# zkh2018/ethsnarks

Hardware: AMD Instinct MI355X
Metric: groth16_proofs_per_sec (higher is better)
Workload: dtype u32 (8-limb 254-bit Montgomery integers)

## Files before the change

### ethsnarks_amd/csrc/bn254.hpp

```cpp
#pragma once
#include "common.hpp"
#include <stdint.h>
#if defined(__HIP_DEVICE_COMPILE__) && !defined(ZK_NO_ASM)
#include "fips_asm.hpp"
#endif

#ifndef ZK_HD
#define ZK_HD __host__ __device__ __forceinline__
#endif
#define ZK_HD_NOINLINE __host__ __device__ __attribute__((noinline))

namespace zk {

struct alignas(16) fe { uint32_t l[8]; };

struct FrParams {
    static ZK_HD constexpr uint32_t p(int i) {
        constexpr uint32_t v[8] = {0xf0000001u, 0x43e1f593u, 0x79b97091u, 0x2833e848u, 0x8181585du, 0xb85045b6u, 0xe131a029u, 0x30644e72u};
        return v[i];
    }
    static ZK_HD constexpr uint32_t one(int i) {
        constexpr uint32_t v[8] = {0x4ffffffbu, 0xac96341cu, 0x9f60cd29u, 0x36fc7695u, 0x7879462eu, 0x666ea36fu, 0x9a07df2fu, 0x0e0a77c1u};
        return v[i];
    }
// ... 335 lines not shown
#endif
    static ZK_HD void lmul_pair(const fe &a, const fe &b, const fe &c, const fe &d, fe &r0, fe &r1) { lmul_x2(a, b, c, d, r0, r1); }
    static ZK_HD void lsqr_pair(const fe &a, const fe &b, fe &r0, fe &r1) { lmul_pair(a, a, b, b, r0, r1); }
    static ZK_HD fe lsqr(const fe &a) { return lmul(a, a); }
    static ZK_HD fe ldbl(const fe &a) { return ladd(a, a); }
    static ZK_HD fe lneg(const fe &a) { return lsub(zero(), a); }
#if defined(__HIP_DEVICE_COMPILE__) && !defined(ZK_NO_ASM)
    static __device__ __forceinline__ fe lneg_op(const fe &a) {
        fe pp, d;
#pragma unroll
        for (int i = 0; i < 8; i++) pp.l[i] = (P::p(i) << 1) | (i ? P::p(i - 1) >> 31 : 0u);
        fips::sub8(d.l, pp.l, a.l);
        return d;
    }
#else
    static ZK_HD fe lneg_op(const fe &a) { return lneg(a); }
#endif
    static ZK_HD fe lneg_yop(const fe &a) { return lneg(a); }
    static ZK_HD fe qsel(uint32_t ql, const fe &a, const fe &b, const fe &c, const fe &d) {
        fe r; const bool odd = ql & 1u, hi = ql & 2u;
#pragma unroll
        for (int i = 0; i < 8; i++) { const uint32_t x = odd ? b.l[i] : a.l[i], y = odd ? d.l[i] : c.l[i]; r.l[i] = hi ? y : x; }
        return r;
    }
#if defined(__HIP_DEVICE_COMPILE__) && !defined(ZK_NO_ASM)
    template <int S> static __device__ __forceinline__ fe qbcast(const fe &v) {
        fe r;
#pragma unroll
        for (int i = 0; i < 8; i++) r.l[i] = (uint32_t)__builtin_amdgcn_update_dpp(0, (int)v.l[i], S * 0x55, 0xf, 0xf, false);
        return r;
    }
#endif
    static ZK_HD fe canon(const fe &a) { return reduce_once(a); }

    static ZK_HD fe to_mont(const fe &a) { fe r2; for (int i = 0; i < 8; i++) r2.l[i] = P::r2(i); return mul(a, r2); }
    static ZK_HD fe from_mont(const fe &a) { fe o = zero(); o.l[0] = 1; return mul(a, o); }

    static ZK_HD fe pow(const fe &a, const uint32_t e[8]) {
        fe acc = one(), base = a;
        for (int i = 0; i < 256; i++) {
            if ((e[i >> 5] >> (i & 31)) & 1) acc = mul(acc, base);
            base = sqr(base);
        }
        return acc;
    }
    static ZK_HD fe pow_u64(const fe &a, uint64_t e) {
        fe acc = one(), base = a;
        while (e) { if (e & 1) acc = mul(acc, base); base = sqr(base); e >>= 1; }
        return acc;
    }
    static ZK_HD fe inv(const fe &a) {
        uint32_t e[8];
        for (int i = 0; i < 8; i++) e[i] = P::p(i);
        e[0] -= 2;
        return pow(a, e);
    }
    static ZK_HD fe from_u64(uint64_t v) { fe t = zero(); t.l[0] = (uint32_t)v; t.l[1] = (uint32_t)(v >> 32); return to_mont(t); }
};

typedef Field<FrParams> Fr;
typedef Field<FqParams> Fq;

struct alignas(16) fe2 { fe c0, c1; };

struct Fq2 {
    typedef fe2 elem;
    static ZK_HD fe2 zero() { fe2 r; r.c0 = Fq::zero(); r.c1 = Fq::zero(); return r; }
    static ZK_HD fe2 one() { fe2 r; r.c0 = Fq::one(); r.c1 = Fq::zero(); return r; }
    static ZK_HD bool is_zero(const fe2 &a) { return Fq::is_zero(a.c0) && Fq::is_zero(a.c1); }
    static ZK_HD bool eq(const fe2 &a, const fe2 &b) { return Fq::eq(a.c0, b.c0) && Fq::eq(a.c1, b.c1); }
    static ZK_HD fe2 add(const fe2 &a, const fe2 &b) { fe2 r; r.c0 = Fq::add(a.c0, b.c0); r.c1 = Fq::add(a.c1, b.c1); return r; }
    static ZK_HD fe2 sub(const fe2 &a, const fe2 &b) { fe2 r; r.c0 = Fq::sub(a.c0, b.c0); r.c1 = Fq::sub(a.c1, b.c1); return r; }
    static ZK_HD fe2 neg(const fe2 &a) { fe2 r; r.c0 = Fq::neg(a.c0); r.c1 = Fq::neg(a.c1); return r; }
    static ZK_HD fe2 dbl(const fe2 &a) { return add(a, a); }
    static ZK_HD fe2 mul(const fe2 &a, const fe2 &b) {
        fe v0 = Fq::mul(a.c0, b.c0), v1 = Fq::mul(a.c1, b.c1);
        fe s = Fq::mul(Fq::add(a.c0, a.c1), Fq::add(b.c0, b.c1));
        fe2 r; r.c0 = Fq::sub(v0, v1); r.c1 = Fq::sub(Fq::sub(s, v0), v1); return r;
    }
    static ZK_HD fe2 sqr(const fe2 &a) {
        fe p = Fq::mul(a.c0, a.c1);
        fe2 r; r.c0 = Fq::mul(Fq::add(a.c0, a.c1), Fq::sub(a.c0, a.c1)); r.c1 = Fq::add(p, p); return r;
    }
    static ZK_HD bool lis_zero(const fe2 &a) { return Fq::lis_zero(a.c0) && Fq::lis_zero(a.c1); }
    static ZK_HD fe2 ladd(const fe2 &a, const fe2 &b) { fe2 r; r.c0 = Fq::ladd(a.c0, b.c0); r.c1 = Fq::ladd(a.c1, b.c1); return r; }
    static ZK_HD fe2 lsub(const fe2 &a, const fe2 &b) { fe2 r; r.c0 = Fq::lsub(a.c0, b.c0); r.c1 = Fq::lsub(a.c1, b.c1); return r; }
    static ZK_HD fe2 lneg(const fe2 &a) { fe2 r; r.c0 = Fq::lneg(a.c0); r.c1 = Fq::lneg(a.c1); return r; }
    static ZK_HD fe2 lneg_op(const fe2 &a) { fe2 r; r.c0 = Fq::lneg_op(a.c0); r.c1 = Fq::lneg_op(a.c1); return r; }
    static ZK_HD fe2 lneg_yop(const fe2 &a) { return lneg_op(a); }
    static ZK_HD fe2 ldbl(const fe2 &a) { return ladd(a, a); }
    static ZK_HD fe2 lmul(const fe2 &a, const fe2 &b) {
        fe2 r;
        r.c0 = Fq::lmul2(a.c0, b.c0, a.c1, Fq::lneg_op(b.c1));
        r.c1 = Fq::lmul2(a.c0, b.c1, a.c1, b.c0);
        return r;
    }
    static constexpr bool PAIRS = false;
    static ZK_HD void lmul_pair(const fe2 &a, const fe2 &b, const fe2 &c, const fe2 &d, fe2 &r0, fe2 &r1) { r0 = lmul(a, b); r1 = lmul(c, d); }
    static ZK_HD void lsqr_pair(const fe2 &a, const fe2 &b, fe2 &r0, fe2 &r1) { r0 = lsqr(a); r1 = lsqr(b); }
    static ZK_HD fe2 lmul2(const fe2 &a, const fe2 &b, const fe2 &c, const fe2 &d) {
        fe2 r;
        r.c0 = Fq::lmul4(a.c0, b.c0, a.c1, Fq::lneg_op(b.c1), c.c0, d.c0, c.c1, Fq::lneg_op(d.c1));
        r.c1 = Fq::lmul4(a.c0, b.c1, a.c1, b.c0, c.c0, d.c1, c.c1, d.c0);
        return r;
    }
    static ZK_HD fe2 lsqr(const fe2 &a) {
        fe p = Fq::lmul(a.c0, a.c1);
        fe2 r; r.c0 = Fq::lmul(Fq::ladd(a.c0, a.c1), Fq::lsub(a.c0, a.c1)); r.c1 = Fq::ladd(p, p); return r;
    }
    static ZK_HD fe2 canon(const fe2 &a) { fe2 r; r.c0 = Fq::canon(a.c0); r.c1 = Fq::canon(a.c1); return r; }
    static ZK_HD fe2 qsel(uint32_t ql, const fe2 &a, const fe2 &b, const fe2 &c, const fe2 &d) {
        fe2 r; r.c0 = Fq::qsel(ql, a.c0, b.c0, c.c0, d.c0); r.c1 = Fq::qsel(ql, a.c1, b.c1, c.c1, d.c1); return r;
    }
#if defined(__HIP_DEVICE_COMPILE__) && !defined(ZK_NO_ASM)
    template <int S> static __device__ __forceinline__ fe2 qbcast(const fe2 &v) { fe2 r; r.c0 = Fq::qbcast<S>(v.c0); r.c1 = Fq::qbcast<S>(v.c1); return r; }
#endif
    static ZK_HD fe2 inv(const fe2 &a) {
        fe n = Fq::inv(Fq::add(Fq::sqr(a.c0), Fq::sqr(a.c1)));
        fe2 r; r.c0 = Fq::mul(a.c0, n); r.c1 = Fq::neg(Fq::mul(a.c1, n)); return r;
    }
};

template <class F>
struct Curve {
    typedef typename F::elem E;
    static constexpr int WAVES_PER_SIMD = sizeof(E) > 32 ? 2 : 4;
    static constexpr int WAVES_PER_SIMD_PAIRS = sizeof(E) > 32 ? 2 : 3;
    struct alignas(16) Affine { E x, y; };
    struct alignas(16) XYZZ { E X, Y, ZZ, ZZZ; };

    static ZK_HD bool is_inf(const Affine &p) { return F::lis_zero(p.x) && F::lis_zero(p.y); }
    static ZK_HD bool is_inf(const XYZZ &p) { return F::lis_zero(p.ZZ); }
    static ZK_HD XYZZ infinity() { XYZZ r; r.X = F::zero(); r.Y = F::zero(); r.ZZ = F::zero(); r.ZZZ = F::zero(); return r; }
    static ZK_HD Affine aff_infinity() { Affine r; r.x = F::zero(); r.y = F::zero(); return r; }
    static ZK_HD XYZZ from_affine(const Affine &p) {
        if (is_inf(p)) return infinity();
        XYZZ r; r.X = p.x; r.Y = p.y; r.ZZ = F::one(); r.ZZZ = F::one(); return r;
    }
    static ZK_HD Affine neg(const Affine &p) { Affine r; r.x = p.x; r.y = F::lneg(p.y); return r; }
    static ZK_HD XYZZ neg(const XYZZ &p) { XYZZ r = p; r.Y = F::lneg(p.Y); return r; }

    static ZK_HD XYZZ dbl_affine(const Affine &p) {
        if (is_inf(p)) return infinity();
        E U = F::ldbl(p.y), V = F::lsqr(U), W = F::lmul(U, V), S = F::lmul(p.x, V);
        E xx = F::lsqr(p.x), M = F::ladd(F::ldbl(xx), xx);
        XYZZ r;
        r.X = F::lsub(F::lsqr(M), F::ldbl(S));
        r.Y = F::lmul2(M, F::lsub(S, r.X), W, F::lneg_yop(p.y));
        r.ZZ = V; r.ZZZ = W;
        return r;
    }
    static ZK_HD XYZZ dbl(const XYZZ &p) {
        if (is_inf(p)) return p;
        E U = F::ldbl(p.Y), V = F::lsqr(U), W = F::lmul(U, V), S = F::lmul(p.X, V);
        E xx = F::lsqr(p.X), M = F::ladd(F::ldbl(xx), xx);
        XYZZ r;
        r.X = F::lsub(F::lsqr(M), F::ldbl(S));
        r.Y = F::lmul2(M, F::lsub(S, r.X), W, F::lneg_yop(p.Y));
        r.ZZ = F::lmul(V, p.ZZ); r.ZZZ = F::lmul(W, p.ZZZ);
        return r;
    }
    static ZK_HD XYZZ madd(const XYZZ &p, const Affine &q) {
        if (is_inf(q)) return p;
        if (is_inf(p)) { XYZZ r; r.X = q.x; r.Y = q.y; r.ZZ = F::one(); r.ZZZ = F::one(); return r; }
        E U2 = F::lmul(q.x, p.ZZ), S2 = F::lmul(q.y, p.ZZZ);
        E Pd = F::lsub(U2, p.X), R = F::lsub(S2, p.Y);
        if (F::lis_zero(Pd)) {
            if (F::lis_zero(R)) return dbl_affine(q);
            return infinity();
        }
        XYZZ r;
        const E PP = F::lsqr(Pd);
        r.ZZ = F::lmul(p.ZZ, PP);
        const E Q = F::lmul(p.X, PP), PPP = F::lmul(Pd, PP);
        r.ZZZ = F::lmul(p.ZZZ, PPP);
        r.X = F::lsub(F::lsub(F::lsqr(R), PPP), F::ldbl(Q));
        r.Y = F::lmul2(R, F::lsub(Q, r.X), F::lneg_yop(p.Y), PPP);
        return r;
    }
    static ZK_HD XYZZ madd_pairs(const XYZZ &p, const Affine &q) {
        if constexpr (!F::PAIRS) return madd(p, q);
        else {
        if (is_inf(q)) return p;
        if (is_inf(p)) { XYZZ r; r.X = q.x; r.Y = q.y; r.ZZ = F::one(); r.ZZZ = F::one(); return r; }
        E U2, S2;
        F::lmul_pair(q.x, p.ZZ, q.y, p.ZZZ, U2, S2);
        E Pd = F::lsub(U2, p.X), R = F::lsub(S2, p.Y);
        if (F::lis_zero(Pd)) {
            if (F::lis_zero(R)) return dbl_affine(q);
            return infinity();
        }
        XYZZ r;
        E PP, RR, Q, PPP;
        F::lsqr_pair(Pd, R, PP, RR);
        F::lmul_pair(p.X, PP, Pd, PP, Q, PPP);
        F::lmul_pair(p.ZZ, PP, p.ZZZ, PPP, r.ZZ, r.ZZZ);
        r.X = F::lsub(F::lsub(RR, PPP), F::ldbl(Q));
        r.Y = F::lmul2(R, F::lsub(Q, r.X), F::lneg_yop(p.Y), PPP);
        return r;
        }
    }
    static ZK_HD XYZZ add(const XYZZ &p, const XYZZ &q) {
        if (is_inf(p)) return q;
        if (is_inf(q)) return p;
        E U1 = F::lmul(p.X, q.ZZ), U2 = F::lmul(q.X, p.ZZ);
        E S1 = F::lmul(p.Y, q.ZZZ), S2 = F::lmul(q.Y, p.ZZZ);
        E Pd = F::lsub(U2, U1), R = F::lsub(S2, S1);
        if (F::lis_zero(Pd)) {
            if (F::lis_zero(R)) return dbl(p);
            return infinity();
        }
        E PP = F::lsqr(Pd), PPP = F::lmul(Pd, PP), Q = F::lmul(U1, PP);
        XYZZ r;
        r.X = F::lsub(F::lsub(F::lsqr(R), PPP), F::ldbl(Q));
        r.Y = F::lmul2(R, F::lsub(Q, r.X), F::lneg_yop(S1), PPP);
        r.ZZ = F::lmul(F::lmul(p.ZZ, q.ZZ), PP); r.ZZZ = F::lmul(F::lmul(p.ZZZ, q.ZZZ), PPP);
        return r;
    }
#if defined(__HIP_DEVICE_COMPILE__) && !defined(ZK_NO_ASM)
#define ZK_QB(S, v) F::template qbcast<S>(v)
    static __device__ __forceinline__ XYZZ dbl_q(const XYZZ &p, uint32_t ql) {
        if (is_inf(p)) return p;
        const E U = F::ldbl(p.Y);
        E a = F::qsel(ql, U, p.X, U, U);
        E t = F::lmul(a, a);
        const E V = ZK_QB(0, t), xx = ZK_QB(1, t), M = F::ladd(F::ldbl(xx), xx);
        t = F::lmul(F::qsel(ql, U, p.X, M, V), F::qsel(ql, V, V, M, p.ZZ));
        const E W = ZK_QB(0, t), S = ZK_QB(1, t), MM = ZK_QB(2, t);
        XYZZ r; r.ZZ = ZK_QB(3, t);
        r.X = F::lsub(MM, F::ldbl(S));
        t = F::lmul(F::qsel(ql, M, W, W, W), F::qsel(ql, F::lsub(S, r.X), p.Y, p.ZZZ, p.ZZZ));
        r.Y = F::lsub(ZK_QB(0, t), ZK_QB(1, t)); r.ZZZ = ZK_QB(2, t);
        return r;
    }
    static __device__ __forceinline__ XYZZ add_q(const XYZZ &p, const XYZZ &q, uint32_t ql) {
        if (is_inf(p)) return q;
        if (is_inf(q)) return p;
        E t = F::lmul(F::qsel(ql, p.X, q.X, p.Y, q.Y), F::qsel(ql, q.ZZ, p.ZZ, q.ZZZ, p.ZZZ));
        const E U1 = ZK_QB(0, t), U2 = ZK_QB(1, t), S1 = ZK_QB(2, t), S2 = ZK_QB(3, t);
        const E Pd = F::lsub(U2, U1), R = F::lsub(S2, S1);
        if (F::lis_zero(Pd)) {
            if (F::lis_zero(R)) return dbl_q(p, ql);
            return infinity();
        }
        t = F::lmul(F::qsel(ql, Pd, R, p.ZZ, p.ZZZ), F::qsel(ql, Pd, R, q.ZZ, q.ZZZ));
        const E PP = ZK_QB(0, t), RR = ZK_QB(1, t), ZZ12 = ZK_QB(2, t), ZZZ12 = ZK_QB(3, t);
        t = F::lmul(F::qsel(ql, Pd, U1, ZZ12, ZZ12), PP);
        const E PPP = ZK_QB(0, t), Q = ZK_QB(1, t);
        XYZZ r; r.ZZ = ZK_QB(2, t);
        r.X = F::lsub(F::lsub(RR, PPP), F::ldbl(Q));
        t = F::lmul(F::qsel(ql, R, S1, ZZZ12, ZZZ12), F::qsel(ql, F::lsub(Q, r.X), PPP, PPP, PPP));
        r.Y = F::lsub(ZK_QB(0, t), ZK_QB(1, t)); r.ZZZ = ZK_QB(2, t);
        return r;
    }
    static __device__ __forceinline__ XYZZ madd_q(const XYZZ &p, const Affine &q, uint32_t ql) {
        if (is_inf(q)) return p;
        if (is_inf(p)) { XYZZ r; r.X = q.x; r.Y = q.y; r.ZZ = F::one(); r.ZZZ = F::one(); return r; }
        E t = F::lmul(F::qsel(ql, q.x, q.y, q.x, q.y), F::qsel(ql, p.ZZ, p.ZZZ, p.ZZ, p.ZZZ));
        const E Pd = F::lsub(ZK_QB(0, t), p.X), R = F::lsub(ZK_QB(1, t), p.Y);
        if (F::lis_zero(Pd)) {
            if (F::lis_zero(R)) return dbl_affine(q);
            return infinity();
        }
        E a = F::qsel(ql, Pd, R, Pd, R);
        t = F::lmul(a, a);
        const E PP = ZK_QB(0, t), RR = ZK_QB(1, t);
        t = F::lmul(F::qsel(ql, Pd, p.X, p.ZZ, p.ZZ), PP);
        const E PPP = ZK_QB(0, t), Q = ZK_QB(1, t);
        XYZZ r; r.ZZ = ZK_QB(2, t);
        r.X = F::lsub(F::lsub(RR, PPP), F::ldbl(Q));
        t = F::lmul(F::qsel(ql, R, p.Y, p.ZZZ, p.ZZZ), F::qsel(ql, F::lsub(Q, r.X), PPP, PPP, PPP));
        r.Y = F::lsub(ZK_QB(0, t), ZK_QB(1, t)); r.ZZZ = ZK_QB(2, t);
        return r;
    }
#undef ZK_QB
#else
    static ZK_HD XYZZ dbl_q(const XYZZ &p, uint32_t) { return dbl(p); }
    static ZK_HD XYZZ add_q(const XYZZ &p, const XYZZ &q, uint32_t) { return add(p, q); }
    static ZK_HD XYZZ madd_q(const XYZZ &p, const Affine &q, uint32_t) { return madd(p, q); }
#endif
    template <int Q> static ZK_HD XYZZ addQ(const XYZZ &p, const XYZZ &q, uint32_t ql) { if constexpr (Q == 4) return add_q(p, q, ql); else return add(p, q); }
    template <int Q> static ZK_HD XYZZ dblQ(const XYZZ &p, uint32_t ql) { if constexpr (Q == 4) return dbl_q(p, ql); else return dbl(p); }
    template <int Q> static ZK_HD XYZZ maddQ(const XYZZ &p, const Affine &q, uint32_t ql) { if constexpr (Q == 4) return madd_q(p, q, ql); else return madd(p, q); }
    template <int Q> static ZK_HD XYZZ maddV(const XYZZ &p, const Affine &q, uint32_t ql) { if constexpr (Q == 2) return madd_pairs(p, q); else return maddQ<Q>(p, q, ql); }

    static ZK_HD XYZZ canon(const XYZZ &p) { XYZZ r; r.X = F::canon(p.X); r.Y = F::canon(p.Y); r.ZZ = F::canon(p.ZZ); r.ZZZ = F::canon(p.ZZZ); return r; }
    static ZK_HD Affine to_affine(const XYZZ &p) {
        if (is_inf(p)) return aff_infinity();
        const XYZZ c = canon(p);
        E i = F::inv(F::mul(c.ZZ, c.ZZZ));
        E izz = F::mul(i, c.ZZZ), izzz = F::mul(i, c.ZZ);
        Affine r; r.x = F::mul(c.X, izz); r.y = F::mul(c.Y, izzz); return r;
    }
};

typedef Curve<Fq> G1;
typedef Curve<Fq2> G2;

}
```

### ethsnarks_amd/csrc/msm.hpp

```cpp
#pragma once
#include "bn254.hpp"
#include "common.hpp"
#include <stdlib.h>

namespace zk {

constexpr uint32_t MSM_SEG_MIN = 32;
constexpr uint32_t MSM_SEG_MIN_SMALL = 8;
constexpr uint32_t MSM_SEG_MAX = 48;
constexpr uint32_t MSM_HEAVY = 64;
constexpr uint32_t MSM_TREE = 256;
constexpr uint32_t MSM_HEAVY_GRID = 256;

constexpr uint32_t SORT_THREADS = 256;
constexpr uint32_t SORT_FINE_THREADS = 1024;
constexpr uint32_t SORT_MAX_CB = 256;
constexpr uint32_t SORT_MAX_FB = 4096;
constexpr uint32_t SORT_STAGE = 7680;
static_assert(SORT_MAX_CB == SORT_THREADS, "k_sort_partition_staged: one coarse bin per thread");

struct SortShape {
    uint32_t cb, fb, fine_bits, groups, per_group;
    void set(uint32_t n, uint32_t nb, uint32_t W = 15) {
        per_group = 512;
        while (per_group > 32 && (uint64_t)per_group * W > SORT_STAGE) per_group >>= 1;
        if (const char *e = getenv("ZK_SORT_PER_GROUP")) { int v = atoi(e); if (v >= 64) per_group = (uint32_t)v; }
        resize(n, nb);
    }
    void resize(uint32_t n, uint32_t nb) {
        fine_bits = 0; while (((nb + (1u << fine_bits) - 1) >> fine_bits) > SORT_MAX_CB) fine_bits++;
        fb = 1u << fine_bits;
        cb = (nb + fb - 1) >> fine_bits;
        groups = (n + per_group - 1) / per_group; if (!groups) groups = 1;
    }
};

struct ChunkRule {
    uint32_t slots = 1, seg_min = MSM_SEG_MIN, seg_max = MSM_SEG_MAX;
    ZK_HD uint32_t len(uint32_t total) const {
        if ((uint64_t)seg_min * slots >= total) return seg_min;
        const uint64_t per_round = (uint64_t)seg_max * slots;
        const uint64_t rounds = (total + per_round - 1) / per_round, lanes = rounds * slots;
        const uint32_t seg = (uint32_t)((total + lanes - 1) / lanes);
        return seg < seg_min ? seg_min : seg;
    }
    uint64_t max_chunks(uint64_t entries_bound) const { return entries_bound / seg_max + slots + 1; }
};
inline uint32_t msm_machine_threads(uint32_t waves_per_simd) {
#ifdef ZK_EMUL
    return 32 * waves_per_simd;
#else
    int dev = 0, cus = 0;
    if (hipGetDevice(&dev) != hipSuccess || hipDeviceGetAttribute(&cus, hipDeviceAttributeMultiprocessorCount, dev) != hipSuccess || cus <= 0) cus = 256;
    return (uint32_t)cus * 4u * waves_per_simd * 64u;
#endif
}

struct MsmShape {
    uint32_t n = 0, c = 0, W = 0, nb = 0;
    uint32_t plog = 0;
    ZK_HD uint32_t planes() const { return 1u << plog; }
    ZK_HD uint32_t rows() const { return (W + planes() - 1) >> plog; }
    ZK_HD uint32_t lo_bits() const { return c / 2; }
    ZK_HD uint32_t hi_bits() const { return (c - 1) - c / 2; }
    ChunkRule chunk;
    uint32_t quad = 1;
    uint32_t quad_acc = 1;
    bool acc_pairs = false;
    uint32_t rowcol_seg = 16;
    static uint32_t pick_c(uint32_t n, uint32_t batch = 1) {
        for (uint32_t c = 17; c > 2; c--) {
            const uint64_t entries = (uint64_t)n * (254 / c + 1);
            const uint64_t floor_c = c >= 16 ? 2 * MSM_SEG_MIN - 1 : MSM_SEG_MIN;
            uint64_t per_bucket = floor_c;
            if (batch > 1) {
                per_bucket = 32 * entries * batch / 1482910;
                if (per_bucket > 100) per_bucket = 100;
                if (per_bucket < floor_c) per_bucket = floor_c;
            }
            if (entries >= (per_bucket << (c - 1))) return c;
        }
        return 2;
    }
    void set(uint32_t n_, uint32_t c_, uint32_t batch = 1, uint32_t plog_ = 0) {
        plog = plog_;
        n = n_; c = c_ ? c_ : pick_c(n_, batch ? batch : 1);
        if (c < 2) c = 2;
        if (c > 20) c = 20;
        W = 254 / c + 1; nb = 1u << (c - 1);
        const uint64_t all = max_entries() * (batch ? batch : 1);
        quad = all <= (1ull << 21) ? 4 : 1;
        quad_acc = all <= (1ull << 17) ? 4 : 1;
        if (const char *e = getenv("ZK_MSM_QUAD")) quad = atoi(e) ? 4 : 1;
        if (const char *e = getenv("ZK_MSM_QUAD_ACC")) quad_acc = atoi(e) ? 4 : 1;
        acc_pairs = all >= (3ull << 21);
        if (const char *e = getenv("ZK_ACC_PAIRS")) acc_pairs = atoi(e) != 0;
        if (const char *e = getenv("ZK_ROWCOL_SEG")) { int v = atoi(e); if (v >= 1 && v <= 256 && !(v & (v - 1))) rowcol_seg = (uint32_t)v; }
        chunk.seg_min = all <= (1ull << 23) ? MSM_SEG_MIN_SMALL : MSM_SEG_MIN;
        chunk.seg_max = MSM_SEG_MAX;
        if (const char *e = getenv("ZK_SEG_MIN")) { int v = atoi(e); if (v >= 4) chunk.seg_min = (uint32_t)v; }
        if (const char *e = getenv("ZK_SEG_MAX")) { int v = atoi(e); if (v >= 4) chunk.seg_max = (uint32_t)v; }
        if (chunk.seg_max < chunk.seg_min) chunk.seg_max = chunk.seg_min;
    }
    void set_slots(uint32_t waves_per_simd) { chunk.slots = msm_machine_threads(waves_per_simd) / quad_acc; if (!chunk.slots) chunk.slots = 1; }
    uint64_t max_entries() const { return (uint64_t)n * W; }
    uint64_t max_chunks() const { return chunk.max_chunks(max_entries()); }
    uint64_t max_pieces() const { return max_chunks() + nb + 1; }
};

struct SortView {
    const uint32_t *sorted = nullptr, *off = nullptr;
    uint32_t nb = 0, entries_bound = 0;
    uint32_t batch = 1;
    uint32_t remap_src = 0, remap_offset = 0;
    uint32_t remap_kbits = 0;
    const uint32_t *remap_pos = nullptr;
};

template <class C>
struct MsmWork {
    MsmShape sh;
    SortShape ss;
    uint32_t max_batch = 1;
    uint32_t cur_batch = 1;
    typename C::Affine *table = nullptr;
    uint32_t table_n = 0;
    bool owns_table = true;
    uint2 *pairs = nullptr;
    uint32_t *counts = nullptr, *bin_total = nullptr, *bin_base = nullptr;
    uint32_t *off = nullptr, *sorted = nullptr;
    uint32_t *heavy_list = nullptr, *heavy_count = nullptr;
    typename C::XYZZ *pieces = nullptr, *bucket = nullptr, *partial_a = nullptr, *partial_b = nullptr;
    typename C::XYZZ *host_result = nullptr;
    typename C::XYZZ *dev_result = nullptr;
    size_t dev_result_pitch = 0;
    hipEvent_t ev_acc0 = nullptr, ev_acc1 = nullptr;
    float accumulate_ms() const { float ms = 0; if (ev_acc0 && ev_acc1) hipEventElapsedTime(&ms, ev_acc0, ev_acc1); return ms; }

    int alloc(uint32_t n, uint32_t c, typename C::Affine *shared_table = nullptr, const MsmShape *sort_like = nullptr, bool sort_only = false, uint32_t batch = 1, uint32_t plog = 0);
    void release();
    int precompute(const typename C::Affine *d_bases, uint32_t n, hipStream_t st);
    int enqueue(const fe *scalars, const uint32_t *gather, uint32_t n, int canonical, hipStream_t st, hipStream_t st_tail, uint32_t batch = 1, uint32_t stride = 0);
    int enqueue_sort(const fe *scalars, const uint32_t *gather, uint32_t n, int canonical, hipStream_t st, uint32_t batch = 1, uint32_t stride = 0);
    int enqueue_reduce(const SortView &v, hipStream_t st, hipStream_t st_tail, uint32_t tail_lanes = 0);
    int enqueue_accumulate(const SortView &v, hipStream_t st);
    int enqueue_tail(hipStream_t st_tail, uint32_t tail_lanes = 0, MsmWork *also = nullptr);
    bool tail_pending = false;
    template <int Q> int launch_reduce(hipStream_t st, const MsmWork *also);
    const uint32_t *cur_off = nullptr;
    uint32_t sort_batch = 1;
    uint32_t sort_kbits = 0;
    void use_shift_payload() { uint32_t k = 1; while ((1ull << k) < table_n) k++; if (((uint64_t)sh.rows() << k) < (1ull << 31)) sort_kbits = k; }
    SortView view() const { SortView v; v.sorted = sorted; v.off = off; v.batch = sort_batch << sh.plog; v.nb = sh.nb * v.batch; v.entries_bound = (uint32_t)((uint64_t)table_n * sh.W * sort_batch); return v; }
    SortView view_for(uint32_t offset, const uint32_t *pos = nullptr) const { SortView v = view(); v.remap_src = table_n; v.remap_offset = offset; v.remap_pos = pos; v.remap_kbits = sort_kbits; return v; }
    typename C::XYZZ finish(uint32_t proof = 0) const {
        const uint32_t S = sh.planes();
        typename C::XYZZ r = C::canon(host_result[(size_t)proof * S + (S - 1)]);
        for (uint32_t j = S - 1; j-- > 0;) {
            for (uint32_t d = 0; d < sh.c; d++) r = C::dbl(r);
            r = C::add(r, C::canon(host_result[(size_t)proof * S + j]));
        }
        return S > 1 ? C::canon(r) : r;
    }
};

}
```

### ethsnarks_amd/csrc/msm_impl.hpp

```cpp
#pragma once
#include "msm.hpp"
#include <string.h>

namespace zk {

template <class C>
__global__ void __launch_bounds__(64, C::WAVES_PER_SIMD)
k_msm_precompute(const typename C::Affine *__restrict__ bases, uint32_t n, uint32_t c, uint32_t W,
                 typename C::Affine *__restrict__ table) {
    uint32_t k = blockIdx.x * blockDim.x + threadIdx.x;
    if (k >= n) return;
    const typename C::Affine p = bases[k];
    table[k] = p;
    typename C::XYZZ cur = C::from_affine(p);
    for (uint32_t w = 1; w < W; w++) {
        for (uint32_t j = 0; j < c; j++) cur = C::dbl(cur);
        table[(size_t)w * n + k] = C::to_affine(cur);
    }
}

static ZK_D uint32_t msm_digit(const fe &s, uint32_t w, uint32_t c, uint32_t &carry, uint32_t &neg) {
    const uint32_t nb = 1u << (c - 1), full = 1u << c;
    uint32_t bit = w * c, limb = bit >> 5, off = bit & 31;
    uint32_t lo = 0, hi = 0;
#pragma unroll
    for (uint32_t k = 0; k < 8; k++) { if (k == limb) lo = s.l[k]; if (k == limb + 1) hi = s.l[k]; }
    uint64_t v = lo | ((uint64_t)hi << 32);
    uint32_t d = ((uint32_t)(v >> off) & (full - 1)) + carry;
    neg = 0; carry = 0;
    if (d > nb) { d = full - d; neg = 1; carry = 1; }
    return d;
}
static ZK_D fe msm_load_scalar(const fe *__restrict__ scalars, const uint32_t *__restrict__ gather, uint32_t p, uint32_t stride, uint32_t il, int canonical) {
    fe s = scalars[(size_t)p * stride + (gather ? gather[il] : il)];
    return canonical ? s : Fr::from_mont(s);
}

template <class C>
__global__ void __launch_bounds__(SORT_THREADS)
k_sort_count(const fe *__restrict__ scalars, const uint32_t *__restrict__ gather, uint32_t n, uint32_t batch, uint32_t stride, int canonical,
             uint32_t c, uint32_t W, uint32_t plog, SortShape ss, uint32_t *__restrict__ counts) {
    __shared__ uint32_t cnt[SORT_MAX_CB];
    for (uint32_t k = threadIdx.x; k < ss.cb; k += blockDim.x) cnt[k] = 0;
    __syncthreads();
    const uint32_t total = n * batch, nbp = 1u << (c - 1);
    const uint32_t i0 = blockIdx.x * ss.per_group, i1 = (i0 + ss.per_group < total) ? i0 + ss.per_group : total;
    for (uint32_t i = i0 + threadIdx.x; i < i1; i += blockDim.x) {
        const uint32_t p = i / n, il = i - p * n;
        const fe s = msm_load_scalar(scalars, gather, p, stride, il, canonical);
        uint32_t carry = 0, neg;
        for (uint32_t w = 0; w < W; w++) {
            uint32_t d = msm_digit(s, w, c, carry, neg);
            if (d) atomicAdd(&cnt[((((p << plog) | (w & ((1u << plog) - 1u))) * nbp) + d - 1) >> ss.fine_bits], 1u);
        }
    }
    __syncthreads();
    for (uint32_t k = threadIdx.x; k < ss.cb; k += blockDim.x) counts[(size_t)k * ss.groups + blockIdx.x] = cnt[k];
}

template <class C>
__global__ void __launch_bounds__(SORT_THREADS)
k_sort_colscan(uint32_t *__restrict__ counts, uint32_t groups, uint32_t *__restrict__ bin_total) {
    __shared__ uint32_t sh[SORT_THREADS];
    uint32_t *row = counts + (size_t)blockIdx.x * groups;
    const uint32_t t = threadIdx.x, per = (groups + SORT_THREADS - 1) / SORT_THREADS;
    const uint32_t g0 = t * per, g1 = (g0 + per < groups) ? g0 + per : groups;
    uint32_t sum = 0;
    for (uint32_t g = g0; g < g1; g++) sum += row[g];
    sh[t] = sum;
    __syncthreads();
    for (uint32_t d = 1; d < SORT_THREADS; d <<= 1) {
        uint32_t v = (t >= d) ? sh[t - d] : 0;
        __syncthreads();
        sh[t] += v;
        __syncthreads();
    }
    uint32_t e = sh[t] - sum;
    for (uint32_t g = g0; g < g1; g++) { uint32_t v = row[g]; row[g] = e; e += v; }
    if (t == SORT_THREADS - 1) bin_total[blockIdx.x] = sh[t];
}

template <class C>
__global__ void __launch_bounds__(SORT_THREADS)
k_sort_binscan(const uint32_t *__restrict__ bin_total, uint32_t cb, uint32_t *__restrict__ bin_base) {
    __shared__ uint32_t sh[SORT_THREADS];
    const uint32_t t = threadIdx.x, v0 = t < cb ? bin_total[t] : 0;
    sh[t] = v0;
    __syncthreads();
    for (uint32_t d = 1; d < SORT_THREADS; d <<= 1) {
        uint32_t v = (t >= d) ? sh[t - d] : 0;
        __syncthreads();
        sh[t] += v;
        __syncthreads();
    }
    if (t < cb) bin_base[t] = sh[t] - v0;
    if (t == SORT_THREADS - 1) bin_base[cb] = sh[t];
}

template <class C>
__global__ void __launch_bounds__(SORT_THREADS)
k_sort_partition(const fe *__restrict__ scalars, const uint32_t *__restrict__ gather, uint32_t n, uint32_t batch, uint32_t stride, int canonical,
                 uint32_t c, uint32_t W, uint32_t plog, SortShape ss, const uint32_t *__restrict__ counts,
                 const uint32_t *__restrict__ bin_base, uint2 *__restrict__ pairs, uint32_t kbits) {
    __shared__ uint32_t pos[SORT_MAX_CB];
    for (uint32_t k = threadIdx.x; k < ss.cb; k += blockDim.x) pos[k] = bin_base[k] + counts[(size_t)k * ss.groups + blockIdx.x];
    __syncthreads();
    const uint32_t total = n * batch, nbp = 1u << (c - 1);
    const uint32_t i0 = blockIdx.x * ss.per_group, i1 = (i0 + ss.per_group < total) ? i0 + ss.per_group : total;
    for (uint32_t i = i0 + threadIdx.x; i < i1; i += blockDim.x) {
        const uint32_t pr = i / n, il = i - pr * n;
        const fe s = msm_load_scalar(scalars, gather, pr, stride, il, canonical);
        uint32_t carry = 0, neg;
        for (uint32_t w = 0; w < W; w++) {
            uint32_t d = msm_digit(s, w, c, carry, neg);
            if (!d) continue;
            const uint32_t b = ((pr << plog) | (w & ((1u << plog) - 1u))) * nbp + d - 1;
            uint32_t p = atomicAdd(&pos[b >> ss.fine_bits], 1u);
            const uint32_t row = w >> plog;
            uint2 e; e.x = (kbits ? (row << kbits) | il : row * n + il) | (neg << 31); e.y = b;
            pairs[p] = e;
        }
    }
}

template <class C>
__global__ void __launch_bounds__(SORT_THREADS)
k_sort_partition_staged(const fe *__restrict__ scalars, const uint32_t *__restrict__ gather, uint32_t n, uint32_t batch, uint32_t stride, int canonical,
                        uint32_t c, uint32_t W, uint32_t plog, SortShape ss, const uint32_t *__restrict__ counts, const uint32_t *__restrict__ bin_total,
                        const uint32_t *__restrict__ bin_base, uint2 *__restrict__ pairs, uint32_t kbits) {
    __shared__ uint2 stage[SORT_STAGE];
    __shared__ uint32_t lbase[SORT_MAX_CB], lcur[SORT_MAX_CB], gpos[SORT_MAX_CB], scan[SORT_THREADS];
    const uint32_t t = threadIdx.x, g = blockIdx.x;
    uint32_t cnt = 0;
    if (t < ss.cb) {
        const uint32_t cur = counts[(size_t)t * ss.groups + g], nxt = g + 1 < ss.groups ? counts[(size_t)t * ss.groups + g + 1] : bin_total[t];
        cnt = nxt - cur; gpos[t] = bin_base[t] + cur;
    }
    scan[t] = cnt;
    __syncthreads();
    for (uint32_t d = 1; d < SORT_THREADS; d <<= 1) {
        const uint32_t v = t >= d ? scan[t - d] : 0;
        __syncthreads();
        scan[t] += v;
        __syncthreads();
    }
    lbase[t] = lcur[t] = scan[t] - cnt;
    const uint32_t local_total = scan[SORT_THREADS - 1];
    __syncthreads();
    const uint32_t total = n * batch, nbp = 1u << (c - 1);
    const uint32_t i0 = g * ss.per_group, i1 = (i0 + ss.per_group < total) ? i0 + ss.per_group : total;
    for (uint32_t i = i0 + t; i < i1; i += blockDim.x) {
        const uint32_t pr = i / n, il = i - pr * n;
        const fe sc = msm_load_scalar(scalars, gather, pr, stride, il, canonical);
        uint32_t carry = 0, neg;
        for (uint32_t w = 0; w < W; w++) {
            uint32_t d = msm_digit(sc, w, c, carry, neg);
            if (!d) continue;
            const uint32_t b = ((pr << plog) | (w & ((1u << plog) - 1u))) * nbp + d - 1;
            const uint32_t row = w >> plog;
            uint2 e; e.x = (kbits ? (row << kbits) | il : row * n + il) | (neg << 31); e.y = b;
            stage[atomicAdd(&lcur[b >> ss.fine_bits], 1u)] = e;
        }
    }
    __syncthreads();
    for (uint32_t sl = t; sl < local_total; sl += blockDim.x) {
        const uint2 e = stage[sl];
        const uint32_t bin = e.y >> ss.fine_bits;
        pairs[gpos[bin] + (sl - lbase[bin])] = e;
    }
}

template <class C>
__global__ void __launch_bounds__(SORT_FINE_THREADS)
k_sort_fine(const uint2 *__restrict__ pairs, const uint32_t *__restrict__ bin_base, SortShape ss, uint32_t nb,
            uint32_t *__restrict__ off, uint32_t *__restrict__ sorted) {
    __shared__ uint32_t cnt[SORT_MAX_FB], cur[SORT_MAX_FB], sh[SORT_FINE_THREADS];
    const uint32_t bin = blockIdx.x, r0 = bin_base[bin], r1 = bin_base[bin + 1], t = threadIdx.x, T = blockDim.x;
    const uint32_t fmask = ss.fb - 1;
    for (uint32_t k = t; k < ss.fb; k += T) cnt[k] = 0;
    __syncthreads();
    for (uint32_t e = r0 + t; e < r1; e += 4 * T) {
        uint32_t y[4];
#pragma unroll
        for (uint32_t u = 0; u < 4; u++) y[u] = e + u * T < r1 ? pairs[e + u * T].y : 0xffffffffu;
#pragma unroll
        for (uint32_t u = 0; u < 4; u++) if (e + u * T < r1) atomicAdd(&cnt[y[u] & fmask], 1u);
    }
    __syncthreads();
    const uint32_t per = (ss.fb + T - 1) / T, k0 = t * per, k1 = (k0 + per < ss.fb) ? k0 + per : ss.fb;
    uint32_t sum = 0;
    for (uint32_t k = k0; k < k1; k++) sum += cnt[k];
    sh[t] = sum;
    __syncthreads();
    for (uint32_t d = 1; d < T; d <<= 1) {
        uint32_t v = (t >= d) ? sh[t - d] : 0;
        __syncthreads();
        sh[t] += v;
        __syncthreads();
    }
    uint32_t ex = sh[t] - sum;
    for (uint32_t k = k0; k < k1; k++) {
        const uint32_t b = bin * ss.fb + k;
        if (b < nb) off[b] = r0 + ex;
        cur[k] = r0 + ex;
        ex += cnt[k];
    }
    if (bin + 1 == gridDim.x && t == 0) off[nb] = r1;
    __syncthreads();
    for (uint32_t e = r0 + t; e < r1; e += 4 * T) {
        uint2 pr[4];
#pragma unroll
        for (uint32_t u = 0; u < 4; u++) if (e + u * T < r1) pr[u] = pairs[e + u * T];
#pragma unroll
        for (uint32_t u = 0; u < 4; u++) if (e + u * T < r1) sorted[atomicAdd(&cur[pr[u].y & fmask], 1u)] = pr[u].x;
    }
}

template <class C, int Q>
__global__ void __launch_bounds__(64, Q == 2 ? C::WAVES_PER_SIMD_PAIRS : C::WAVES_PER_SIMD)
k_msm_accumulate(const typename C::Affine *__restrict__ table, const uint32_t *__restrict__ sorted,
                 const uint32_t *__restrict__ off, uint32_t nb, ChunkRule rule,
                 uint32_t remap_src, uint32_t remap_offset, const uint32_t *__restrict__ remap_pos, uint32_t n_dst, uint32_t remap_kbits,
                 typename C::XYZZ *__restrict__ piece) {
    constexpr uint32_t LANES = Q == 4 ? 4 : 1;
    const uint32_t gt = blockIdx.x * blockDim.x + threadIdx.x, c = gt / LANES, ql = gt % LANES;
    const uint32_t total = off[nb], seg = rule.len(total);
    if ((uint64_t)c * seg >= total) return;
    const uint32_t begin = c * seg, end = (total - begin < seg) ? total : begin + seg;
    uint32_t lo = 0, hi = nb;
    while (hi - lo > 1) { uint32_t mid = (lo + hi) >> 1; if (off[mid] <= begin) lo = mid; else hi = mid; }
    uint32_t b = lo, bucket_end = off[b + 1];
    typename C::XYZZ acc = C::infinity();
    constexpr bool PREFETCH_POINT = sizeof(typename C::Affine) <= 64;
    auto entry_index = [&](uint32_t p) -> uint32_t {
        uint32_t idx = p & 0x7fffffffu;
        if (remap_src) {
            uint32_t w, i;
            if (remap_kbits) { w = idx >> remap_kbits; i = idx & ((1u << remap_kbits) - 1u); }
            else { w = idx / remap_src; i = idx - w * remap_src; }
            const uint32_t k = remap_pos ? remap_pos[i] : i - remap_offset;
            if (k >= n_dst) return 0xffffffffu;
            idx = w * n_dst + k;
        }
        return idx;
    };
    uint32_t p_next = sorted[begin];
    typename C::Affine q_next = C::aff_infinity();
    if constexpr (PREFETCH_POINT) {
        const uint32_t idx = entry_index(p_next); if (idx != 0xffffffffu) q_next = table[idx];
    }
    for (uint32_t e = begin; e < end; e++) {
        if (e >= bucket_end) {
            if (ql == 0) piece[c + b] = acc;
            acc = C::infinity();
            do { b++; bucket_end = off[b + 1]; } while (e >= bucket_end);
        }
        const uint32_t p = p_next;
        typename C::Affine q;
        if constexpr (PREFETCH_POINT) {
            q = q_next;
            if (e + 1 < end) {
                p_next = sorted[e + 1];
                const uint32_t idx = entry_index(p_next);
                q_next = C::aff_infinity();
                if (idx != 0xffffffffu) q_next = table[idx];
            }
        } else {
            if (e + 1 < end) p_next = sorted[e + 1];
            const uint32_t idx = entry_index(p);
            if (idx == 0xffffffffu) continue;
            q = table[idx];
        }
        if (p >> 31) q = C::neg(q);
        acc = C::template maddV<Q>(acc, q, ql);
    }
    if (ql == 0) piece[c + b] = acc;
}

struct PieceRange { uint32_t s0, s1; ZK_HD uint32_t n() const { return s1 - s0; } };
static ZK_D PieceRange msm_piece_range(const uint32_t *__restrict__ off, uint32_t nb, const ChunkRule &rule, uint32_t b) {
    const uint32_t e0 = off[b], e1 = off[b + 1], seg = rule.len(off[nb]);
    PieceRange r; r.s0 = r.s1 = 0;
    if (e1 > e0) { r.s0 = e0 / seg + b; r.s1 = (e1 - 1) / seg + b + 1; }
    return r;
}
template <class C, int Q>
__global__ void __launch_bounds__(64, C::WAVES_PER_SIMD / 2)
k_msm_bucket_finalize(const typename C::XYZZ *__restrict__ piece, const uint32_t *__restrict__ off,
                      uint32_t nb, ChunkRule rule,
                      const typename C::XYZZ *__restrict__ piece2, const uint32_t *__restrict__ off2, ChunkRule rule2,
                      typename C::XYZZ *__restrict__ bucket,
                      uint32_t *__restrict__ heavy_list, uint32_t *__restrict__ heavy_count) {
    const uint32_t gt = blockIdx.x * blockDim.x + threadIdx.x, b = gt / Q, ql = gt % Q;
    if (b >= nb) return;
    const PieceRange r1 = msm_piece_range(off, nb, rule, b);
    PieceRange r2; r2.s0 = r2.s1 = 0;
    if (piece2) r2 = msm_piece_range(off2, nb, rule2, b);
    if (r1.n() + r2.n() > MSM_HEAVY) { if (ql == 0) heavy_list[atomicAdd(heavy_count, 1u)] = b; return; }
    typename C::XYZZ acc = C::infinity();
    for (uint32_t s = r1.s0; s < r1.s1; s++) acc = C::template addQ<Q>(acc, piece[s], ql);
    for (uint32_t s = r2.s0; s < r2.s1; s++) acc = C::template addQ<Q>(acc, piece2[s], ql);
    if (ql == 0) bucket[b] = acc;
}

template <class C, int Q>
__global__ void __launch_bounds__(128 * Q)
k_msm_heavy(const typename C::XYZZ *__restrict__ piece, const uint32_t *__restrict__ off, uint32_t nb, ChunkRule rule,
            const typename C::XYZZ *__restrict__ piece2, const uint32_t *__restrict__ off2, ChunkRule rule2,
            const uint32_t *__restrict__ heavy_list, const uint32_t *__restrict__ heavy_count,
            typename C::XYZZ *__restrict__ bucket) {
    __shared__ typename C::XYZZ sh[64];
    const uint32_t nheavy = *heavy_count, lt = threadIdx.x / Q, ql = threadIdx.x % Q;
    for (uint32_t h = blockIdx.x; h < nheavy; h += gridDim.x) {
        const uint32_t b = heavy_list[h];
        const PieceRange r1 = msm_piece_range(off, nb, rule, b);
        PieceRange r2; r2.s0 = r2.s1 = 0;
        if (piece2) r2 = msm_piece_range(off2, nb, rule2, b);
        typename C::XYZZ acc = C::infinity();
        for (uint32_t i = lt; i < r1.n() + r2.n(); i += 128)
            acc = C::template addQ<Q>(acc, i < r1.n() ? piece[r1.s0 + i] : piece2[r2.s0 + (i - r1.n())], ql);
        for (uint32_t half = 64; half > 0; half >>= 1) {
            if (lt >= half && lt < 2 * half && ql == 0) sh[lt - half] = acc;
            __syncthreads();
            if (lt < half) acc = C::template addQ<Q>(acc, sh[lt], ql);
            __syncthreads();
        }
        if (threadIdx.x == 0) bucket[b] = acc;
    }
}

template <class C, int Q>
__global__ void __launch_bounds__(MSM_TREE)
k_msm_rowcol_sum(const typename C::XYZZ *__restrict__ bucket, uint32_t lo_bits, uint32_t hi_bits, uint32_t seg_row, uint32_t seg_col, uint32_t row_groups,
                 typename C::XYZZ *__restrict__ rc) {
    constexpr uint32_t T = MSM_TREE / Q;
    __shared__ typename C::XYZZ sh[T / 2];
    const uint32_t L = 1u << lo_bits, H = 1u << hi_bits;
    bucket += ((size_t)blockIdx.y << (lo_bits + hi_bits)); rc += (size_t)blockIdx.y * (H + L);
    const uint32_t lt = threadIdx.x / Q, ql = threadIdx.x % Q;
    const bool row = blockIdx.x < row_groups;
    const uint32_t seg = row ? seg_row : seg_col, per = T / seg;
    const uint32_t line = (row ? blockIdx.x : blockIdx.x - row_groups) * per + lt / seg, k = lt % seg;
    const uint32_t n = row ? L : H, lines = row ? H : L;
    const bool live = line < lines;
    const uint32_t first = row ? line << lo_bits : line, step = row ? 1u : L;
    typename C::XYZZ acc = C::infinity();
    if (live) for (uint32_t i = k; i < n; i += seg) acc = C::template addQ<Q>(acc, bucket[first + (size_t)i * step], ql);
    for (uint32_t half = seg / 2; half > 0; half >>= 1) {
        if (k >= half && k < 2 * half && ql == 0) sh[(lt / seg) * (seg / 2) + (k - half)] = acc;
        __syncthreads();
        if (k < half) acc = C::template addQ<Q>(acc, sh[(lt / seg) * (seg / 2) + k], ql);
        __syncthreads();
    }
    if (live && k == 0 && ql == 0) rc[row ? line : H + line] = acc;
}

template <class C, int Q>
__global__ void __launch_bounds__(MSM_TREE)
k_msm_weighted_sum(const typename C::XYZZ *__restrict__ rc, uint32_t lo_bits, uint32_t hi_bits, typename C::XYZZ *__restrict__ out) {
    constexpr uint32_t TH = MSM_TREE / Q / 2;
    __shared__ typename C::XYZZ sh[2 * TH];
    const uint32_t L = 1u << lo_bits, H = 1u << hi_bits;
    rc += (size_t)blockIdx.x * (H + L);
    const uint32_t lt = threadIdx.x / Q, ql = threadIdx.x % Q, half = lt / TH, t = lt % TH;
    const uint32_t n = half ? L : H;
    const typename C::XYZZ *X = rc + (half ? H : 0);
    typename C::XYZZ *mine = sh + half * TH;
    const uint32_t W = n < TH ? n : TH;
    const uint32_t Wmax = (L > H ? L : H) < TH ? (L > H ? L : H) : TH;
    const uint32_t E = n / W, i0 = t * E;
    typename C::XYZZ run = C::infinity(), acc = C::infinity();
    if (t < W) for (uint32_t e = E; e-- > 0;) {
        run = C::template addQ<Q>(run, X[i0 + e], ql);
        if (e) acc = C::template addQ<Q>(acc, run, ql);
    }
    typename C::XYZZ suf = run;
    if (ql == 0) mine[t] = suf;
    __syncthreads();
    for (uint32_t d = 1; d < Wmax; d <<= 1) {
        typename C::XYZZ other = C::infinity();
        if (t + d < W) other = mine[t + d];
        __syncthreads();
        if (t < W && d < W) { suf = C::template addQ<Q>(suf, other, ql); if (ql == 0) mine[t] = suf; }
        __syncthreads();
    }
    const typename C::XYZZ total = mine[0];
    __syncthreads();
    typename C::XYZZ v = (t && t < W) ? suf : C::infinity();
    for (uint32_t e = E; e > 1; e >>= 1) v = C::template dblQ<Q>(v, ql);
    v = C::template addQ<Q>(v, acc, ql);
    for (uint32_t h = Wmax / 2; h > 0; h >>= 1) {
        if (t >= h && t < 2 * h && ql == 0) mine[t - h] = v;
        __syncthreads();
        if (t < h) v = C::template addQ<Q>(v, mine[t], ql);
        __syncthreads();
    }
    if (t == 0) {
        if (half == 0) for (uint32_t b = 0; b < lo_bits; b++) v = C::template dblQ<Q>(v, ql);
        else v = C::template addQ<Q>(v, total, ql);
        if (ql == 0) mine[0] = v;
    }
    __syncthreads();
    if (lt == 0) {
        v = C::template addQ<Q>(v, sh[TH], ql);
        if (ql == 0) out[blockIdx.x] = v;
    }
}

template <class C>
int MsmWork<C>::alloc(uint32_t n, uint32_t c, typename C::Affine *shared_table, const MsmShape *sort_like, bool sort_only, uint32_t batch, uint32_t plog) {
    max_batch = batch ? batch : 1;
    if (sort_like) sh = *sort_like; else sh.set(n ? n : 1, c, max_batch, plog);
    sh.set_slots(sh.acc_pairs && C::WAVES_PER_SIMD_PAIRS != C::WAVES_PER_SIMD ? C::WAVES_PER_SIMD_PAIRS : C::WAVES_PER_SIMD);
    const uint64_t B = max_batch, BS = (uint64_t)max_batch << sh.plog;
    if ((uint64_t)sh.n * sh.rows() >= (1ull << 31)) return fail_msg(ZK_ERR_ARG, "MSM too large: n * table rows must stay below 2^31 (entry payload = table index | sign)");
    if (sh.max_entries() * B >= (1ull << 32) - 64) return fail_msg(ZK_ERR_ARG, "MSM too large: proofs * n * windows must stay below 2^32 (32-bit entry offsets)");
    if ((uint64_t)sh.nb * BS > (uint64_t)SORT_MAX_CB * SORT_MAX_FB) return fail_msg(ZK_ERR_ARG, "batch too large: proofs * planes * buckets exceeds the sort's 2^20 buckets");
    if (sort_only) { owns_table = false; table_n = n; }
    else if (shared_table) { table = shared_table; owns_table = false; table_n = n; }
    else ZK_HIP(hipMalloc(&table, sizeof(typename C::Affine) * (size_t)(n ? n : 1) * sh.rows()));
    ss.set((uint32_t)(sh.n * B), (uint32_t)(sh.nb * BS), sh.W);
    if (!sort_like) {
        ZK_HIP(hipMalloc(&pairs, sizeof(uint2) * sh.max_entries() * B));
        ZK_HIP(hipMalloc(&counts, sizeof(uint32_t) * ((size_t)SORT_MAX_CB * ss.groups + 1)));
        ZK_HIP(hipMalloc(&bin_total, sizeof(uint32_t) * (SORT_MAX_CB + 1)));
        ZK_HIP(hipMalloc(&bin_base, sizeof(uint32_t) * (SORT_MAX_CB + 1)));
        ZK_HIP(hipMalloc(&sorted, sizeof(uint32_t) * sh.max_entries() * B));
        ZK_HIP(hipMalloc(&off, sizeof(uint32_t) * (sh.nb * BS + 1)));
    }
    if (sort_only) return ZK_OK;
    const uint64_t n_pieces = sh.chunk.max_chunks(sh.max_entries() * B) + sh.nb * BS + 1;
    ZK_HIP(hipMalloc(&heavy_list, sizeof(uint32_t) * sh.nb * BS));
    ZK_HIP(hipMalloc(&heavy_count, sizeof(uint32_t)));
    ZK_HIP(hipMalloc(&pieces, sizeof(typename C::XYZZ) * n_pieces));
    ZK_HIP(hipMalloc(&bucket, sizeof(typename C::XYZZ) * sh.nb * BS));
    const uint32_t rowcol = (1u << sh.lo_bits()) + (1u << sh.hi_bits());
    ZK_HIP(hipMalloc(&partial_a, sizeof(typename C::XYZZ) * ((size_t)rowcol * BS + 1)));
    ZK_HIP(hipMalloc(&partial_b, sizeof(typename C::XYZZ) * (BS + 1)));
    ZK_HIP(hipHostMalloc(&host_result, sizeof(typename C::XYZZ) * BS, hipHostMallocDefault));
    ZK_HIP(hipEventCreate(&ev_acc0)); ZK_HIP(hipEventCreate(&ev_acc1));
    return ZK_OK;
}

template <class C>
void MsmWork<C>::release() {
    if (!owns_table) table = nullptr;
    void *dev[] = {table, pairs, counts, bin_total, bin_base, off, sorted, heavy_list, heavy_count, pieces, bucket, partial_a, partial_b};
    for (void *p : dev) if (p) hipFree(p);
    if (host_result) hipHostFree(host_result);
    if (ev_acc0) hipEventDestroy(ev_acc0);
    if (ev_acc1) hipEventDestroy(ev_acc1);
    *this = MsmWork();
}

// ... 118 lines not shown
```

Baseline: 115.7.

## Reorder XYZZ dbl/add, widen sort_fine loads, merge finalize loops, retune bounds

The XYZZ doubling and addition are reordered so ZZ/ZZZ products are computed early, and add's equal-point fallback now doubles the normalized point. k_sort_fine drops to 256 threads with 16 loads in flight per thread plus a min-blocks hint, and bucket finalize merges its two piece loops into one with a fixed tail-wave launch bound. The goal is lower register pressure and shorter live ranges in the EC kernels and more memory-level parallelism in the sort, at the cost of possibly lower occupancy or more branches in the merged loop.

```diff
diff --git a/ethsnarks_amd/csrc/bn254.hpp b/ethsnarks_amd/csrc/bn254.hpp
--- a/ethsnarks_amd/csrc/bn254.hpp
+++ b/ethsnarks_amd/csrc/bn254.hpp
@@ -511,12 +511,14 @@
     }
     static ZK_HD XYZZ dbl(const XYZZ &p) {
         if (is_inf(p)) return p;
-        E U = F::ldbl(p.Y), V = F::lsqr(U), W = F::lmul(U, V), S = F::lmul(p.X, V);
-        E xx = F::lsqr(p.X), M = F::ladd(F::ldbl(xx), xx);
         XYZZ r;
+        const E U = F::ldbl(p.Y), V = F::lsqr(U), W = F::lmul(U, V);
+        r.ZZ = F::lmul(V, p.ZZ);
+        const E S = F::lmul(p.X, V);
+        r.ZZZ = F::lmul(W, p.ZZZ);
+        const E xx = F::lsqr(p.X), M = F::ladd(F::ldbl(xx), xx);
         r.X = F::lsub(F::lsqr(M), F::ldbl(S));
         r.Y = F::lmul2(M, F::lsub(S, r.X), W, F::lneg_yop(p.Y));
-        r.ZZ = F::lmul(V, p.ZZ); r.ZZZ = F::lmul(W, p.ZZZ);
         return r;
     }
     static ZK_HD XYZZ madd(const XYZZ &p, const Affine &q) {
@@ -562,18 +564,18 @@
     static ZK_HD XYZZ add(const XYZZ &p, const XYZZ &q) {
         if (is_inf(p)) return q;
         if (is_inf(q)) return p;
-        E U1 = F::lmul(p.X, q.ZZ), U2 = F::lmul(q.X, p.ZZ);
-        E S1 = F::lmul(p.Y, q.ZZZ), S2 = F::lmul(q.Y, p.ZZZ);
-        E Pd = F::lsub(U2, U1), R = F::lsub(S2, S1);
+        const E U1 = F::lmul(p.X, q.ZZ), Pd = F::lsub(F::lmul(q.X, p.ZZ), U1);
+        const E S1 = F::lmul(p.Y, q.ZZZ), R = F::lsub(F::lmul(q.Y, p.ZZZ), S1);
+        const E ZZ12 = F::lmul(p.ZZ, q.ZZ), ZZZ12 = F::lmul(p.ZZZ, q.ZZZ);
         if (F::lis_zero(Pd)) {
-            if (F::lis_zero(R)) return dbl(p);
+            if (F::lis_zero(R)) { XYZZ d; d.X = U1; d.Y = S1; d.ZZ = ZZ12; d.ZZZ = ZZZ12; return dbl(d); }
             return infinity();
         }
-        E PP = F::lsqr(Pd), PPP = F::lmul(Pd, PP), Q = F::lmul(U1, PP);
+        const E PP = F::lsqr(Pd), PPP = F::lmul(Pd, PP), Q = F::lmul(U1, PP);
         XYZZ r;
+        r.ZZ = F::lmul(ZZ12, PP); r.ZZZ = F::lmul(ZZZ12, PPP);
         r.X = F::lsub(F::lsub(F::lsqr(R), PPP), F::ldbl(Q));
         r.Y = F::lmul2(R, F::lsub(Q, r.X), F::lneg_yop(S1), PPP);
-        r.ZZ = F::lmul(F::lmul(p.ZZ, q.ZZ), PP); r.ZZZ = F::lmul(F::lmul(p.ZZZ, q.ZZZ), PPP);
         return r;
     }
 #if defined(__HIP_DEVICE_COMPILE__) && !defined(ZK_NO_ASM)
diff --git a/ethsnarks_amd/csrc/msm.hpp b/ethsnarks_amd/csrc/msm.hpp
--- a/ethsnarks_amd/csrc/msm.hpp
+++ b/ethsnarks_amd/csrc/msm.hpp
@@ -11,9 +11,11 @@
 constexpr uint32_t MSM_HEAVY = 64;
 constexpr uint32_t MSM_TREE = 256;
 constexpr uint32_t MSM_HEAVY_GRID = 256;
+constexpr int MSM_TAIL_WAVES = 2;
 
 constexpr uint32_t SORT_THREADS = 256;
-constexpr uint32_t SORT_FINE_THREADS = 1024;
+constexpr uint32_t SORT_FINE_THREADS = 256;
+constexpr uint32_t SORT_FINE_LOADS = 16;
 constexpr uint32_t SORT_MAX_CB = 256;
 constexpr uint32_t SORT_MAX_FB = 4096;
 constexpr uint32_t SORT_STAGE = 7680;
diff --git a/ethsnarks_amd/csrc/msm_impl.hpp b/ethsnarks_amd/csrc/msm_impl.hpp
--- a/ethsnarks_amd/csrc/msm_impl.hpp
+++ b/ethsnarks_amd/csrc/msm_impl.hpp
@@ -171,20 +171,21 @@
 }
 
 template <class C>
-__global__ void __launch_bounds__(SORT_FINE_THREADS)
+__global__ void __launch_bounds__(SORT_FINE_THREADS, 8)
 k_sort_fine(const uint2 *__restrict__ pairs, const uint32_t *__restrict__ bin_base, SortShape ss, uint32_t nb,
             uint32_t *__restrict__ off, uint32_t *__restrict__ sorted) {
+    constexpr uint32_t U = SORT_FINE_LOADS;
     __shared__ uint32_t cnt[SORT_MAX_FB], cur[SORT_MAX_FB], sh[SORT_FINE_THREADS];
     const uint32_t bin = blockIdx.x, r0 = bin_base[bin], r1 = bin_base[bin + 1], t = threadIdx.x, T = blockDim.x;
     const uint32_t fmask = ss.fb - 1;
     for (uint32_t k = t; k < ss.fb; k += T) cnt[k] = 0;
     __syncthreads();
-    for (uint32_t e = r0 + t; e < r1; e += 4 * T) {
-        uint32_t y[4];
+    for (uint32_t e = r0 + t; e < r1; e += U * T) {
+        uint32_t y[U];
 #pragma unroll
-        for (uint32_t u = 0; u < 4; u++) y[u] = e + u * T < r1 ? pairs[e + u * T].y : 0xffffffffu;
+        for (uint32_t u = 0; u < U; u++) y[u] = e + u * T < r1 ? pairs[e + u * T].y : 0xffffffffu;
 #pragma unroll
-        for (uint32_t u = 0; u < 4; u++) if (e + u * T < r1) atomicAdd(&cnt[y[u] & fmask], 1u);
+        for (uint32_t u = 0; u < U; u++) if (e + u * T < r1) atomicAdd(&cnt[y[u] & fmask], 1u);
     }
     __syncthreads();
     const uint32_t per = (ss.fb + T - 1) / T, k0 = t * per, k1 = (k0 + per < ss.fb) ? k0 + per : ss.fb;
@@ -207,12 +208,12 @@
     }
     if (bin + 1 == gridDim.x && t == 0) off[nb] = r1;
     __syncthreads();
-    for (uint32_t e = r0 + t; e < r1; e += 4 * T) {
-        uint2 pr[4];
+    for (uint32_t e = r0 + t; e < r1; e += U * T) {
+        uint2 pr[U];
 #pragma unroll
-        for (uint32_t u = 0; u < 4; u++) if (e + u * T < r1) pr[u] = pairs[e + u * T];
+        for (uint32_t u = 0; u < U; u++) if (e + u * T < r1) pr[u] = pairs[e + u * T];
 #pragma unroll
-        for (uint32_t u = 0; u < 4; u++) if (e + u * T < r1) sorted[atomicAdd(&cur[pr[u].y & fmask], 1u)] = pr[u].x;
+        for (uint32_t u = 0; u < U; u++) if (e + u * T < r1) sorted[atomicAdd(&cur[pr[u].y & fmask], 1u)] = pr[u].x;
     }
 }
 
@@ -285,7 +286,7 @@
     return r;
 }
 template <class C, int Q>
-__global__ void __launch_bounds__(64, C::WAVES_PER_SIMD / 2)
+__global__ void __launch_bounds__(64, MSM_TAIL_WAVES)
 k_msm_bucket_finalize(const typename C::XYZZ *__restrict__ piece, const uint32_t *__restrict__ off,
                       uint32_t nb, ChunkRule rule,
                       const typename C::XYZZ *__restrict__ piece2, const uint32_t *__restrict__ off2, ChunkRule rule2,
@@ -297,9 +298,10 @@
     PieceRange r2; r2.s0 = r2.s1 = 0;
     if (piece2) r2 = msm_piece_range(off2, nb, rule2, b);
     if (r1.n() + r2.n() > MSM_HEAVY) { if (ql == 0) heavy_list[atomicAdd(heavy_count, 1u)] = b; return; }
+    const uint32_t n1 = r1.n(), n = n1 + r2.n();
+    const typename C::XYZZ *src1 = piece + r1.s0, *src2 = piece2 + r2.s0 - n1;
     typename C::XYZZ acc = C::infinity();
-    for (uint32_t s = r1.s0; s < r1.s1; s++) acc = C::template addQ<Q>(acc, piece[s], ql);
-    for (uint32_t s = r2.s0; s < r2.s1; s++) acc = C::template addQ<Q>(acc, piece2[s], ql);
+    for (uint32_t i = 0; i < n; i++) acc = C::template addQ<Q>(acc, (i < n1 ? src1 : src2)[i], ql);
     if (ql == 0) bucket[b] = acc;
 }
 
```

After: 115.7, median of 6. Within noise of the previous version (+0.0%).
